# Orca0917/TransformerTTS

Measured on AMD Instinct MI355X. Metric: mel frames/sec teacher-forced step, LJSpeech-shape batch, 1/2/4/8 MI355X, higher is better.
Workload: dtype f32; 1 GPU; BASELINE configs[2] (batch 64, 1 GPU; per-GPU shard of configs[3]): training step (no-grad fwd + fwd + loss + bwd + clip + Adam), batch 64/GPU x 870 frames x 100 phonemes (dense), base config d_model 256, 3+3 layers, dropout on, fp32; global_batch=64, parallelism=dp1, batch_stream=one resident batch, accumulate=1, process_group=none, grad_allreduce=none (1 GPU), alignments_written=True, dma_gemms=True, layernorm_images=False, head_images=True, fused_cross_kv=True, wgrad_groups=True, twin_encoder=True, twin_postnet=True

## Files before the change

include/ttts_hip.h:

```cpp
#ifndef TTTS_HIP_H
#define TTTS_HIP_H

#include <stddef.h>
#include <stdint.h>

#ifdef __cplusplus
extern "C" {
#endif

#define TTTS_OK 0
#define TTTS_ERR_INVALID (-1)
#define TTTS_ERR_LAUNCH (-2)

#define TTTS_AMAX_SLOTS 1024

#define TTTS_ACT_NONE 0
#define TTTS_ACT_RELU 1
#define TTTS_ACT_TANH 2

typedef struct ttts_step_state {
    uint64_t seed;
    float lr;
    float p_tf;
    int64_t step;
// ... 46 lines not shown
int64_t ttts_weight_split_units(int64_t rows, int64_t cols, int mode, int channels_per_tap);
int ttts_weight_split_batched(const int64_t* descs, int n, int64_t total_blocks, void* stream);
int ttts_linear_fwd_x6(const float* x, const void* w_planes, const float* bias, const float* residual, float* y,
                       int64_t M, int N, int K, int act, float drop_p, uint64_t seed, const uint64_t* step_seed, int row_shift, int T,
                    void* stream);
int ttts_linear_fwd_h3(const float* x, const void* w_planes, const float* bias, const float* residual, float* y,
                       int64_t M, int N, int K, int act, float drop_p, uint64_t seed, const uint64_t* step_seed, int row_shift,
                       int T, const float* x_amax, float* y_amax_out, void* stream);
int ttts_conv1d_fwd_h3_bn_blocks(int B, int T, int cin, int cout, int taps);
int ttts_conv1d_fwd_h3_bn_chunk_rows(int B, int T, int cin, int cout, int taps);
int ttts_conv1d_fwd_h3(const float* x, const void* planes_fwd, const float* bias, float* y, int B, int T, int cin, int cout,
                       int taps, const float* x_amax, float* bn_partials, void* stream);
int ttts_amax_partials(const float* x, int64_t n, float* partials , void* stream);
int ttts_linear_bwd_data_h3(const float* dy, const void* wt_planes, const float* residual, float* dx, int64_t M, int N,
                            int K, const float* relu_out, float relu_scale, const float* dy_amax, float* dx_amax_out,
                            void* stream);
int ttts_act_image(const float* x, void* image, float* row_inv, int64_t M, int K, void* stream);
int ttts_linear_fwd_h3i(const void* x_image, const float* x_row_inv, const void* w_planes, const float* bias,
                        const float* residual, float* y, int64_t M, int N, int K, int act, float drop_p, uint64_t seed,
                        const uint64_t* step_seed, float* y_amax_out, void* stream);
int ttts_linear_bwd_data_h3i(const void* dy_image, const float* dy_row_inv, const void* wt_planes, const float* residual,
                             float* dx, int64_t M, int N, int K, const float* relu_out, float relu_scale,
                             float* dx_amax_out, void* stream);
int ttts_linear_fwd_h3d(const float* x, const void* w_planes, const float* bias, const float* residual, float* y,
                        int64_t M, int N, int K, int act, float drop_p, uint64_t seed, const uint64_t* step_seed,
                        const float* x_amax, float* y_amax_out, void* stream);
int ttts_linear_bwd_data_h3d(const float* dy, const void* wt_planes, const float* residual, float* dx, int64_t M, int N,
                             int K, const float* relu_out, float relu_scale, const float* dy_amax, float* dx_amax_out,
                             void* stream);
int ttts_linear_fwd_h3d_img(const float* x, const void* w_planes, const float* bias, void* y_image, float* y_row_inv,
                            int64_t M, int N, int K, const float* x_amax, float* y_amax_out, int amax_section_cols,
                            void* stream);
int ttts_head_image(const float* x, int64_t ld_x, void* image, int64_t ld_image, float* row_inv, int64_t M, int N, void* stream);
int ttts_conv1d_bwd_data_h3(const float* dy, const void* planes_bwd, float* dx, int B, int T, int cin, int cout, int taps,
                            const float* dy_amax, void* stream);
int ttts_linear_bwd_data_x6(const float* dy, const void* wt_planes, const float* residual, float* dx, int64_t M, int N,
                            int K, const float* relu_out, float relu_scale, void* stream);
int ttts_conv1d_fwd_x6(const float* x, const void* planes_fwd, const float* bias, float* y, int B, int T, int cin, int cout,
                       int taps, void* stream);
int ttts_conv1d_bwd_data_x6(const float* dy, const void* planes_bwd, float* dx, int B, int T, int cin, int cout, int taps,
                            void* stream);
int ttts_linear_bwd_weight_x6(const float* dy, const float* x, float* dw, float* dbias, float* ws, size_t ws_bytes,
                              int64_t M, int N, int K, int row_shift, int T, int accumulate, ttts_reduce_queue* queue,
                              void* stream);
int ttts_conv1d_bwd_weight_x6(const float* dy, const float* x, float* dw, float* dbias, float* ws, size_t ws_bytes, int B,
                              int T, int cin, int cout, int taps, int accumulate, ttts_reduce_queue* queue, void* stream);
int ttts_linear_bwd_weight_h3(const float* dy, const float* x, float* dw, float* dbias, float* ws, size_t ws_bytes,
                              int64_t M, int N, int K, int row_shift, int T, int accumulate, const float* dy_amax,
                              const float* x_amax, ttts_reduce_queue* queue, void* stream);
int ttts_conv1d_bwd_weight_h3(const float* dy, const float* x, float* dw, float* dbias, float* ws, size_t ws_bytes, int B,
                              int T, int cin, int cout, int taps, int accumulate, const float* dy_amax, const float* x_amax,
                              ttts_reduce_queue* queue, void* stream);
int ttts_wgrad_group_ok(int64_t M, int N, int K, int taps);
int ttts_wgrad_group(int n, const float* const* dy, const float* const* x, float* const* dw, float* const* dbias,
                     float* const* ws, const size_t* ws_bytes, const int64_t* M, const int* N, const int* K, const int* taps,
                     const int* T, const int* row_shift, int accumulate, const float* const* dy_amax, const float* const* x_amax,
                     ttts_reduce_queue* queue, void* stream);
int ttts_linear_bwd_weight_h3_parts(const float* dy, const float* x, float* const* dw_parts, float* const* dbias_parts, int nparts,
                                    float* ws, size_t ws_bytes, int64_t M, int N, int K, int accumulate, const float* dy_amax,
                                    const float* x_amax, ttts_reduce_queue* queue, void* stream);

size_t ttts_conv1d_pack_bytes(int cout, int cin, int taps);
int ttts_conv1d_pack_weight(const float* w, float* w_fwd, float* w_bwd, int cout, int cin, int taps, void* stream);
int ttts_conv1d_fwd(const float* x, const float* w_fwd, const float* bias, float* y, int B, int T, int cin, int cout,
                    int taps, void* stream);
int ttts_conv1d_bwd_data(const float* dy, const float* w_bwd, float* dx, int B, int T, int cin, int cout, int taps,
                         void* stream);
int ttts_conv1d_bwd_weight(const float* dy, const float* x, float* dw, float* dbias, float* ws, size_t ws_bytes, int B,
                           int T, int cin, int cout, int taps, int accumulate, ttts_reduce_queue* queue, void* stream);

size_t ttts_bn_workspace_bytes(int64_t M, int C);
int ttts_bn_train_stats(const float* x, float* mean, float* invstd, float* running_mean, float* running_var,
                        int64_t* num_batches_tracked, float* ws, size_t ws_bytes, int64_t M, int C, float momentum,
                        float eps, void* stream);
int ttts_bn_train_stats_from_partials(const float* partials, int nblk, float* mean, float* invstd, float* running_mean,
                                      float* running_var, int64_t* num_batches_tracked, int C, float momentum, float eps,
                                      void* stream);
int ttts_bn_train_stats_from_partials_rows(const float* partials, int nblk, const float* rows, int n_rows, float* mean,
                                           float* invstd, float* running_mean, float* running_var,
                                           int64_t* num_batches_tracked, int C, float momentum, float eps, void* stream);
int ttts_bn_train_stats_twin(const float* partials_a, int nblk_a, const float* rows_a, int n_rows_a, float* mean_a, float* invstd_a,
                             const float* partials_b, int nblk_b, const float* rows_b, int n_rows_b, float* mean_b, float* invstd_b,
                             float* running_mean, float* running_var, int64_t* num_batches_tracked, int C, float momentum,
                             float eps, void* stream);
int ttts_bn_eval_stats(const float* running_mean, const float* running_var, float* mean, float* invstd, int C, float eps,
                       void* stream);
int ttts_bn_apply_fwd(const float* x, const float* mean, const float* invstd, const float* gamma, const float* beta,
                      float* z, int64_t M, int C, int act, float drop_p, uint64_t seed, const uint64_t* step_seed,
                      float* z_amax_out, void* stream);
int ttts_bn_bwd(const float* dz, const float* x, const float* mean, const float* invstd, const float* gamma,
                const float* beta, float* dx, float* dgamma, float* dbeta, float* ws, size_t ws_bytes, int64_t M, int C,
                int act, float drop_p, uint64_t seed, const uint64_t* step_seed, int accumulate, float* dx_amax_out,
                int batch_stats, void* stream);

int ttts_layernorm_fwd(const float* x, const float* gamma, const float* beta, float* y, float* mean, float* rstd,
                       int64_t M, int d, float eps, float* y_amax_out ,
                       void* y_image_out, float* y_row_inv_out, void* stream);
size_t ttts_layernorm_bwd_workspace_bytes(int d);
int ttts_layernorm_bwd(const float* dy, const float* x, const float* mean, const float* rstd, const float* gamma,
                       float* dx, float* dgamma, float* dbeta, float* ws, size_t ws_bytes, int64_t M, int d,
                       int accumulate, void* dx_image_out ,
                       float* dx_row_inv_out, ttts_reduce_queue* queue, void* stream);
int ttts_layernorm_bwd_drop(const float* dy, const float* x, const float* mean, const float* rstd, const float* gamma,
                            float* dx, float* dgamma, float* dbeta, float* ws, size_t ws_bytes, int64_t M, int d,
                            int accumulate, float* dacc, float drop_p, uint64_t seed, const uint64_t* step_seed,
                            float* dacc_amax, void* dacc_image_out , float* dacc_row_inv_out,
// ... 268 lines not shown
```

transformertts_amd/_lib.py:

```python
from __future__ import annotations

import ctypes
import os
from ctypes import c_char_p, c_float, c_int, c_int64, c_size_t, c_uint64, c_void_p

import torch

_HERE = os.path.dirname(os.path.abspath(__file__))
LIB_PATH = os.environ.get("TTTS_LIB", os.path.join(_HERE, "libttts_hip.so"))

P, I, L, F, U, Z = c_void_p, c_int, c_int64, c_float, c_uint64, c_size_t

SIGNATURES = {
    "ttts_last_error": (c_char_p, []),
    "ttts_abi_version": (I, []),
    "ttts_linear_fwd": (I, [P, P, P, P, P, L, I, I, I, F, U, P, I, I, P]),
    "ttts_linear_bwd_data": (I, [P, P, P, P, L, I, I, P, F, P]),
    "ttts_wgrad_workspace_bytes": (Z, [L, I, I, I]),
    "ttts_linear_bwd_weight": (I, [P, P, P, P, P, Z, L, I, I, I, I, I, P, P]),
    "ttts_split_bytes": (Z, [L, L]),
    "ttts_split_image_bytes": (Z, [L, L, I, I, I]),
    "ttts_gemm_tile_choice": (I, [L, I, I, I]),
    "ttts_weight_split": (I, [P, P, I, I, I, I, I, P]),
    "ttts_weight_split_units": (L, [L, L, I, I]),
    "ttts_weight_split_batched": (I, [P, I, L, P]),
    "ttts_linear_fwd_x6": (I, [P, P, P, P, P, L, I, I, I, F, U, P, I, I, P]),
    "ttts_linear_fwd_h3": (I, [P, P, P, P, P, L, I, I, I, F, U, P, I, I, P, P, P]),
    "ttts_conv1d_fwd_h3": (I, [P, P, P, P, I, I, I, I, I, P, P, P]),
    "ttts_conv1d_fwd_h3_bn_blocks": (I, [I, I, I, I, I]),
    "ttts_conv1d_fwd_h3_bn_chunk_rows": (I, [I, I, I, I, I]),
    "ttts_bn_train_stats_from_partials": (I, [P, I, P, P, P, P, P, I, F, F, P]),
    "ttts_bn_train_stats_from_partials_rows": (I, [P, I, P, I, P, P, P, P, P, I, F, F, P]),
    "ttts_bn_train_stats_twin": (I, [P, I, P, I, P, P, P, I, P, I, P, P, P, P, P, I, F, F, P]),
    "ttts_amax_partials": (I, [P, L, P, P]),
    "ttts_linear_bwd_data_h3": (I, [P, P, P, P, L, I, I, P, F, P, P, P]),
    "ttts_act_image": (I, [P, P, P, L, I, P]),
    "ttts_linear_fwd_h3i": (I, [P, P, P, P, P, P, L, I, I, I, F, U, P, P, P]),
    "ttts_linear_bwd_data_h3i": (I, [P, P, P, P, P, L, I, I, P, F, P, P]),
    "ttts_linear_fwd_h3d": (I, [P, P, P, P, P, L, I, I, I, F, U, P, P, P, P]),
    "ttts_linear_bwd_data_h3d": (I, [P, P, P, P, L, I, I, P, F, P, P, P]),
    "ttts_linear_fwd_h3d_img": (I, [P, P, P, P, P, L, I, I, P, P, I, P]),
    "ttts_head_image": (I, [P, L, P, L, P, L, I, P]),
    "ttts_conv1d_bwd_data_h3": (I, [P, P, P, I, I, I, I, I, P, P]),
    "ttts_linear_bwd_data_x6": (I, [P, P, P, P, L, I, I, P, F, P]),
    "ttts_conv1d_fwd_x6": (I, [P, P, P, P, I, I, I, I, I, P]),
    "ttts_conv1d_bwd_data_x6": (I, [P, P, P, I, I, I, I, I, P]),
    "ttts_linear_bwd_weight_x6": (I, [P, P, P, P, P, Z, L, I, I, I, I, I, P, P]),
    "ttts_conv1d_bwd_weight_x6": (I, [P, P, P, P, P, Z, I, I, I, I, I, I, P, P]),
    "ttts_linear_bwd_weight_h3": (I, [P, P, P, P, P, Z, L, I, I, I, I, I, P, P, P, P]),
    "ttts_conv1d_bwd_weight_h3": (I, [P, P, P, P, P, Z, I, I, I, I, I, I, P, P, P, P]),
    "ttts_linear_bwd_weight_h3_parts": (I, [P, P, P, P, I, P, Z, L, I, I, I, P, P, P, P]),
    "ttts_wgrad_group_ok": (I, [L, I, I, I]),
    "ttts_wgrad_group": (I, [I, P, P, P, P, P, P, P, P, P, P, P, P, I, P, P, P, P]),
    "ttts_conv1d_pack_bytes": (Z, [I, I, I]),
    "ttts_conv1d_pack_weight": (I, [P, P, P, I, I, I, P]),
    "ttts_conv1d_fwd": (I, [P, P, P, P, I, I, I, I, I, P]),
    "ttts_conv1d_bwd_data": (I, [P, P, P, I, I, I, I, I, P]),
    "ttts_conv1d_bwd_weight": (I, [P, P, P, P, P, Z, I, I, I, I, I, I, P, P]),
    "ttts_bn_workspace_bytes": (Z, [L, I]),
    "ttts_bn_train_stats": (I, [P, P, P, P, P, P, P, Z, L, I, F, F, P]),
    "ttts_bn_eval_stats": (I, [P, P, P, P, I, F, P]),
    "ttts_bn_apply_fwd": (I, [P, P, P, P, P, P, L, I, I, F, U, P, P, P]),
    "ttts_bn_bwd": (I, [P, P, P, P, P, P, P, P, P, P, Z, L, I, I, F, U, P, I, P, I, P]),
    "ttts_layernorm_fwd": (I, [P, P, P, P, P, P, L, I, F, P, P, P, P]),
    "ttts_layernorm_bwd_workspace_bytes": (Z, [I]),
    "ttts_layernorm_bwd": (I, [P, P, P, P, P, P, P, P, P, Z, L, I, I, P, P, P, P]),
    "ttts_layernorm_bwd_drop": (I, [P, P, P, P, P, P, P, P, P, Z, L, I, I, P, F, U, P, P, P, P, P, P]),
    "ttts_attention_fwd": (I, [P, P, P, P, P, P, P, I, I, I, I, I, I, I, I, I, F, F, U, P, P]),
    "ttts_attention_fwd_x6": (I, [P, P, P, P, P, P, P, I, I, I, I, I, I, I, I, I, F, F, U, P, P]),
    "ttts_attention_fwd_h3": (I, [P, P, P, P, P, P, P, I, I, I, I, I, I, I, I, I, F, F, U, P, P, P, P, P, P, P]),
    "ttts_attention_bwd": (I, [P, P, P, P, P, P, P, P, P, P, P, I, I, I, I, I, I, I, I, I, I, I, I, F, F, U, P, P]),
    "ttts_attention_bwd_x6": (I, [P, P, P, P, P, P, P, P, P, P, P, I, I, I, I, I, I, I, I, I, I, I, I, F, F, U, P, P]),
    "ttts_attention_bwd_h3": (I, [P, P, P, P, P, P, P, P, P, P, P, I, I, I, I, I, I, I, I, I, I, I, I, F, F, U, P, P, P, P, P, P, P, P, P]),
    "ttts_attention_fwd_img": (I, [P, P, P, P, P, P, P, P, P, P, I, I, I, I, I, I, I, I, I, F, F, U, P, P, P, P, L, L, L, P]),
    "ttts_attention_bwd_img": (I, [P, P, P, P, P, P, P, P, P, P, P, P, P, P, I, I, I, I, I, I, I, I, I, I, I, I, F, F, U, P, P, P, P,
                                   P, I, L, L, L, P]),
    "ttts_attention_fwd_wide": (I, [P, P, P, P, P, P, P, I, I, I, I, I, I, I, I, I, F, F, U, P, P]),
    "ttts_attention_bwd_wide": (I, [P, P, P, P, P, P, P, P, P, P, P, I, I, I, I, I, I, I, I, I, I, I, I, F, F, U, P, P]),
    "ttts_attention_fwd_wide_masked": (I, [P, P, P, P, P, P, P, I, I, I, I, I, I, I, I, I, F, F, U, P, P, L, L, L, P, L, P]),
    "ttts_attention_bwd_wide_masked": (I, [P, P, P, P, P, P, P, P, P, P, P, I, I, I, I, I, I, I, I, I, I, I, I, F, F, U, P, P, L, L, L,
                                           P, L, P]),
    "ttts_attention_bwd_wide_dattn": (I, [P, P, P, P, P, P, P, P, P, P, P, I, I, I, I, I, I, I, I, I, I, I, I, F, F, U, P, P, L, L, L,
                                          P, L, P, P, L, L, L, P]),
    "ttts_guided_attention_fwd": (I, [P, P, P, U, F, I, I, I, I, P, I, I, I, P, P]),
    "ttts_guided_attention_bwd": (I, [P, P, P, U, F, I, I, I, I, I, I, P, P]),
    "ttts_alignment_rowstats": (I, [P, L, L, L, P, P, I, I, I, I, I, I, P, P, P, P]),
    "ttts_alignment_select": (I, [P, P, P, I, I, I, I, I, I, P, P, P]),
    "ttts_alignment_durations_argmax": (I, [P, P, P, P, I, I, I, I, I, P, P, P]),
    "ttts_alignment_mas_workspace_bytes": (Z, [I, I, I]),
    "ttts_alignment_mas": (I, [P, I, L, L, L, P, P, P, I, I, I, I, P, Z, P, P, P]),
    "ttts_dtw_workspace_bytes": (Z, [I, I, I]),
    "ttts_dtw": (I, [P, L, L, P, P, L, L, P, I, I, I, I, I, P, Z, P, P, P, P, P, P]),
    "ttts_audio_tables_bytes": (Z, [I, I, I]),
    "ttts_audio_tables_check": (I, [P, Z, I, I, I, I]),
    "ttts_logmel": (I, [P, L, P, I, I, I, I, I, I, P, F, P, P, P, I, P]),
    "ttts_logmel_stats": (I, [P, P, I, I, I, P, P]),
    "ttts_vocoder_pinv_check": (I, [P, Z, I, I]),
    "ttts_mel_to_magnitude": (I, [P, L, L, P, I, I, I, I, I, P, P, F, P, P, P]),
    "ttts_istft": (I, [P, P, I, I, I, I, P, P, P, P]),
    "ttts_stft_project": (I, [P, L, P, P, I, I, I, I, P, P, P, F, P, P, P]),
    "ttts_resample_table_bytes": (Z, [I, I]),
    "ttts_resample_table_check": (I, [P, Z, I, I, I]),
    "ttts_resample_tile": (I, []),
    "ttts_resample": (I, [P, L, P, I, I, I, I, I, P, P, L, P, P]),
    "ttts_pitch_lags": (I, []),
# ... 103 lines not shown
```

transformertts_amd/csrc/gemm.hip:

```cpp
#include <stdlib.h>

#include "gemm_common.h"

namespace ttts {

#ifndef TTTS_GEMM_BK
#define TTTS_GEMM_BK 16
#endif
#ifndef TTTS_X6_XCD
#define TTTS_X6_XCD 1
#endif
#ifndef TTTS_GEMM_MINWAVES
#define TTTS_GEMM_MINWAVES 3
#endif
constexpr int BK = TTTS_GEMM_BK;
constexpr int KC_LD = BK + 1;


template <int BM, int BN, int WM, int WN, bool A_KC, bool B_KC>
__global__ __launch_bounds__(256, TTTS_GEMM_MINWAVES) void gemm_f32_kernel(GemmArgs g) {
    const uint64_t seed_eff = site_seed(g.seed, g.step_seed);
    constexpr int WTM = BM / WM, WTN = BN / WN;
    constexpr int TM = WTM / 32, TN = WTN / 32;
    static_assert(WM * WN == 4, "4 waves per workgroup");
// ... 794 lines not shown
        for (int kt = kt_begin; kt < kt_end; ++kt) {
            const bool more = (kt + 1) < kt_end;
            if (more) load_tiles(kt + 1);
            compute(buf);
            if (more) store_tiles(buf ^ 1);
            __syncthreads();
            buf ^= 1;
        }
    }

    if (g.colsum != nullptr && blockIdx.x == 0 && ztap == 0) {
        float* fs = reinterpret_cast<float*>(lds);
        __syncthreads();
        if (a_slot) fs[a_rh * BM + a_col] = csum;
        __syncthreads();
        if (tid < BM && m0 + tid < g.M) g.colsum[(long)zsplit * g.M + m0 + tid] = fs[tid] + fs[BM + tid];
    }

    float* C = g.C + (long)z * g.c_zstride;
#pragma unroll
    for (int i = 0; i < TM; ++i)
#pragma unroll
        for (int j = 0; j < TN; ++j) {
            const int col = n0 + wn * WTN + j * 32 + l31;
            const int row0 = m0 + wm * WTM + i * 32;
#pragma unroll
            for (int r = 0; r < 16; ++r) {
                const int row = row0 + acc_row(r, half);
                if (row < g.M && col < g.N) C[(long)row * g.ldc + col] = acc[i][j][r];
            }
        }
}

template <int BM, int BN, int WM, int WN>
static int launch_wgrad_split(const GemmArgs& g, int zdim, hipStream_t stream) {
    dim3 grid(cdiv(g.N, BN), cdiv(g.M, BM), zdim);
    hipLaunchKernelGGL((wgrad_bf16x6_kernel<BM, BN, WM, WN>), grid, dim3(256), 0, stream, g);
    TTTS_LAUNCH_CHECK("wgrad_bf16x6_kernel");
    return TTTS_OK;
}

static int dispatch_wgrad_split(const GemmArgs& g, int zdim, int tile, hipStream_t stream) {
    switch (tile) {
        case TILE_64: return launch_wgrad_split<64, 64, 2, 2>(g, zdim, stream);
        case TILE_128x96: return launch_wgrad_split<128, 96, 4, 1>(g, zdim, stream);
        case TILE_96x128: return launch_wgrad_split<96, 128, 1, 4>(g, zdim, stream);
        default: return launch_wgrad_split<128, 128, 2, 2>(g, zdim, stream);
    }
}

enum WgradForm { WG_F32, WG_X6, WG_H3 };
struct WgradPlan { int tile; int nsplit; int kt_per_split; long tiles; };
struct WgradGroup { int cls; long tiles_total; long nkt_max; };

static long wgrad_target_single(WgradForm f, int tile, long tiles, long nkt) {
    if (f != WG_H3) return 768;
    if (tile == H3_TILE_256) return 256;
    return (tiles > 12 && nkt >= 800) ? 512 : 256;
}

constexpr long WG_GROUP_NKT512 = 200;
static long wgrad_group_many(int cls) { return (cls == 3 || cls == 4) ? 8 : 13; }
static long wgrad_target_group(const WgradGroup& grp) {
    if (grp.cls == 2) return 256;
    return (grp.tiles_total >= wgrad_group_many(grp.cls) && grp.nkt_max >= WG_GROUP_NKT512) ? 512 : 256;
}

static WgradPlan plan_wgrad(int64_t M, int N, int K, int taps, WgradForm f, const WgradGroup* grp = nullptr) {
    WgradPlan p; const long bk = f == WG_H3 ? HBK : BK, nkt = (M + bk - 1) / bk;
    p.tile = (K <= 96) ? TILE_128x96 : TILE_128;
    p.tiles = (long)cdiv(N, 128) * cdiv(K, 128) * taps;
    if (f != WG_F32) {
        if (N <= 64 && K <= 64) { p.tile = TILE_64; p.tiles = (long)cdiv(N, 64) * cdiv(K, 64) * taps; }
        else if (N <= 96 && K > 96) p.tile = TILE_96x128;
    } else if (p.tiles < 16) { p.tile = TILE_64; p.tiles = (long)cdiv(N, 64) * cdiv(K, 64) * taps; }
    if (f == WG_H3) {
        const long tiles256 = (long)cdiv(N, 256) * cdiv(K, 256) * taps;
        if (p.tile == TILE_128 && N >= 256 && K >= 256 && tiles256 >= 3 && nkt >= 800) { p.tile = H3_TILE_256; p.tiles = tiles256; }
    }
    long want = grp ? wgrad_target_group(*grp) / grp->tiles_total : wgrad_target_single(f, p.tile, p.tiles, nkt) / p.tiles;
    if (want < 1) want = 1;
    if (!grp && f != WG_F32 && want > 128) want = 128;
    if (want > nkt) want = nkt;
    long per = (nkt + want - 1) / want;
    if (per < 8 && nkt >= 8) per = 8;
    p.kt_per_split = (int)per;
    p.nsplit = (int)((nkt + per - 1) / per);
    return p;
}

static bool wgrad_use_x6(int N, int K) { return (N >= 128 || N == 80 || N == 96) && (K >= 128 || K == 80 || K == 96) && (N >= 128 || K >= 128); }

static int wgrad_class(int64_t M, int N, int K, int taps, long* tiles = nullptr) {
    if (!(M > 0 && N > 0 && K > 0 && taps >= 1 && taps <= 64 && N % 4 == 0 && K % 4 == 0 && wgrad_use_x6(N, K))) return 0;
    const WgradPlan p = plan_wgrad(M, N, K, taps, WG_H3);
    if (tiles) *tiles = p.tiles;
    if (p.tile == TILE_128) return 1;
    if (p.tile == H3_TILE_256 && N % 256 == 0 && K % 256 == 0) return 2;
    if (p.tile == TILE_128x96) return 3;
    if (p.tile == TILE_96x128) return 4;
    return 0;
}

struct WgradLayout { size_t colsum; size_t floats; };
static WgradLayout wgrad_layout(int nsplit, int N, int K, int taps) {
    const size_t prod = (size_t)nsplit * taps * N * K;
    return {prod, prod + (size_t)nsplit * N};
}

struct WgradProblem {
    const float *dy, *x; float* ws; size_t ws_bytes;
    int64_t M; int N, K, taps;
    int B, T, row_shift;
    const float *dy_amax, *x_amax;
    bool conv = false;
    bool bias = false;
};

static GemmArgs wgrad_args(const WgradProblem& pb, WgradForm f, const WgradPlan& p) {
    GemmArgs g = base_args();
    g.A = pb.dy; g.B = pb.x; g.C = pb.ws; g.M = pb.N; g.N = pb.K; g.K = (int)pb.M;
    g.lda = pb.N; g.ldb = pb.K; g.ldc = pb.K;
    g.a_bytes = (uint32_t)((uint64_t)pb.M * pb.N * 4); g.b_bytes = (uint32_t)((uint64_t)pb.M * pb.K * 4);
    g.T = (pb.conv || pb.row_shift != 0) ? pb.T : 0;
    g.shift0 = pb.conv ? -((pb.taps - 1) / 2) : pb.row_shift; g.shift_step = pb.conv ? 1 : 0;
    g.ztaps = pb.taps; g.kt_per_split = p.kt_per_split; g.c_zstride = (long)pb.N * pb.K;
    g.colsum = pb.bias ? pb.ws + wgrad_layout(p.nsplit, pb.N, pb.K, pb.taps).colsum : nullptr;
    if (f == WG_H3) {
        g.a_amax = pb.dy_amax; g.a_amax_n = H3_AMAX_PARTIALS;
        g.b_amax = pb.x_amax; g.b_amax_n = H3_AMAX_PARTIALS;
    }
    return g;
}

static int wgrad_reduce(const WgradProblem& pb, const WgradPlan& p, const float* colsum, float* const* dw, float* const* dbias, int nparts,
                        bool accumulate, hipStream_t stream, ttts_reduce_queue* queue) {
    if (pb.conv) {
        int rc = launch_conv_wgrad_reduce(pb.ws, dw[0], pb.N, pb.K, pb.taps, p.nsplit, accumulate, stream, queue);
        if (rc == TTTS_OK && colsum) rc = launch_reduce_rows(colsum, pb.N, p.nsplit, pb.N, dbias[0], pb.N, nullptr, accumulate, stream, queue);
        return rc;
    }
    const int Np = pb.N / nparts;
    const long nk = (long)pb.N * pb.K, np = (long)Np * pb.K;
    for (int i = 0; i < nparts; ++i) {
        int rc = launch_reduce_rows_pair(pb.ws + (size_t)i * np, nk, p.nsplit, np, dw[i], colsum ? colsum + (size_t)i * Np : nullptr, pb.N, Np,
                                         colsum ? dbias[i] : nullptr, accumulate, stream, queue);
        if (rc) return rc;
    }
    return TTTS_OK;
}

#define ENTRY_REQUIRE(cond, fmt, ...) TTTS_REQUIRE(cond, "%s: " fmt, name, ##__VA_ARGS__)
static int wgrad_check_operands(const char* name, const WgradProblem& pb) {
    ENTRY_REQUIRE(aligned16(pb.dy) && aligned16(pb.x) && aligned16(pb.ws), "pointers must be 16-byte aligned");
// ... 1 lines not shown
    return TTTS_OK;
}

enum WgradStage2 { WG_PAIR, WG_CONV, WG_PARTS };
static int wgrad_single(const char* name, WgradForm f, WgradStage2 stage, WgradProblem pb, float* const* dw, float* const* dbias,
                        int nparts, int accumulate, ttts_reduce_queue* queue, void* stream) {
    pb.conv = stage == WG_CONV;
    ENTRY_REQUIRE(pb.dy && pb.x && pb.ws && dw && (stage == WG_PARTS || dw[0]), "null pointer");
    ENTRY_REQUIRE(f != WG_H3 || (pb.dy_amax && pb.x_amax), "null pointer: dy_amax and x_amax (partial maxima of dy and x) are required");
    if (pb.conv) {
        ENTRY_REQUIRE(pb.B > 0 && pb.T > 0 && pb.K > 0 && pb.N > 0 && pb.taps > 0 && (pb.taps & 1), "bad dims B=%d T=%d cin=%d cout=%d taps=%d",
                      pb.B, pb.T, pb.K, pb.N, pb.taps);
        ENTRY_REQUIRE((long)pb.B * pb.T < (1L << 31), "B*T too large");
        pb.M = (int64_t)pb.B * pb.T;
    }
    ENTRY_REQUIRE(pb.M > 0 && pb.N > 0 && pb.K > 0 && pb.M < (1LL << 31), "bad dims M=%lld N=%d K=%d", (long long)pb.M, pb.N, pb.K);
    ENTRY_REQUIRE(pb.N % 4 == 0 && pb.K % 4 == 0, "%s=%d and %s=%d must be multiples of 4", pb.conv ? "cout" : "N", pb.N,
                  pb.conv ? "cin" : "K", pb.K);
    if (stage == WG_PARTS)
        ENTRY_REQUIRE(nparts > 0 && nparts <= 64 && pb.N % nparts == 0 && (pb.N / nparts) % 4 == 0,
                      "N=%d does not split in %d blocks of whole float4s", pb.N, nparts);
    if (int rc = wgrad_check_operands(name, pb)) return rc;
    ENTRY_REQUIRE(pb.ws_bytes >= ttts_wgrad_workspace_bytes(pb.M, pb.N, pb.K, pb.taps), "workspace too small");
    ENTRY_REQUIRE(pb.conv || pb.row_shift == 0 || (pb.T > 0 && pb.M % pb.T == 0), "row_shift needs T>0 and M %% T == 0");
    for (int i = 0; i < nparts; ++i) ENTRY_REQUIRE(dw[i] != nullptr, "null destination");
    if (!wgrad_use_x6(pb.N, pb.K)) f = WG_F32;
    pb.bias = dbias != nullptr && dbias[0] != nullptr;
    const WgradPlan p = plan_wgrad(pb.M, pb.N, pb.K, pb.taps, f);
    const GemmArgs g = wgrad_args(pb, f, p);
    const int zdim = p.nsplit * pb.taps;
    const int rc = f == WG_H3 ? dispatch_wgrad_h3(g, zdim, p.tile, (hipStream_t)stream)
           : f == WG_X6 ? dispatch_wgrad_split(g, zdim, p.tile, (hipStream_t)stream)
                        : dispatch_gemm<false, false>(g, zdim, p.tile, (hipStream_t)stream);
    return rc ? rc : wgrad_reduce(pb, p, g.colsum, dw, dbias, nparts, accumulate != 0, (hipStream_t)stream, queue);
}

}

using namespace ttts;

extern "C" {

size_t ttts_wgrad_workspace_bytes(int64_t M, int N, int K, int taps) {
    if (!(M > 0 && N > 0 && K > 0 && taps > 0)) return 0;
    int ns = 0;
    auto cover = [&](WgradForm f, const WgradGroup* grp) { const int n = plan_wgrad(M, N, K, taps, f, grp).nsplit; ns = n > ns ? n : ns; };
    cover(WG_F32, nullptr); cover(WG_X6, nullptr); cover(WG_H3, nullptr);
    long tiles = 0;
    if (const int cls = wgrad_class(M, N, K, taps, &tiles)) {
        const long many = wgrad_group_many(cls);
        const WgradGroup alone = {cls, tiles, (long)((M + HBK - 1) / HBK)}, full = {cls, tiles < many ? many : tiles, WG_GROUP_NKT512};
        cover(WG_H3, &alone); cover(WG_H3, &full);
    }
    return wgrad_layout(ns, N, K, taps).floats * sizeof(float);
}

int ttts_linear_bwd_weight(const float* dy, const float* x, float* dw, float* dbias, float* ws, size_t ws_bytes,
                           int64_t M, int N, int K, int row_shift, int T, int accumulate, ttts_reduce_queue* queue, void* stream) {
    return wgrad_single("linear_bwd_weight", WG_F32, WG_PAIR, {dy, x, ws, ws_bytes, M, N, K, 1, 0, T, row_shift, nullptr, nullptr}, &dw, &dbias, 1,
                        accumulate, queue, stream);
}
int ttts_linear_bwd_weight_x6(const float* dy, const float* x, float* dw, float* dbias, float* ws, size_t ws_bytes,
                              int64_t M, int N, int K, int row_shift, int T, int accumulate, ttts_reduce_queue* queue, void* stream) {
    return wgrad_single("linear_bwd_weight_x6", WG_X6, WG_PAIR, {dy, x, ws, ws_bytes, M, N, K, 1, 0, T, row_shift, nullptr, nullptr}, &dw, &dbias, 1,
                        accumulate, queue, stream);
}
int ttts_linear_bwd_weight_h3(const float* dy, const float* x, float* dw, float* dbias, float* ws, size_t ws_bytes,
                              int64_t M, int N, int K, int row_shift, int T, int accumulate, const float* dy_amax,
                              const float* x_amax, ttts_reduce_queue* queue, void* stream) {
    return wgrad_single("linear_bwd_weight_h3", WG_H3, WG_PAIR, {dy, x, ws, ws_bytes, M, N, K, 1, 0, T, row_shift, dy_amax, x_amax}, &dw, &dbias, 1,
                        accumulate, queue, stream);
}

int ttts_linear_bwd_weight_h3_parts(const float* dy, const float* x, float* const* dw_parts, float* const* dbias_parts, int nparts,
                                    float* ws, size_t ws_bytes, int64_t M, int N, int K, int accumulate, const float* dy_amax,
                                    const float* x_amax, ttts_reduce_queue* queue, void* stream) {
    return wgrad_single("linear_bwd_weight_h3_parts", WG_H3, WG_PARTS, {dy, x, ws, ws_bytes, M, N, K, 1, 0, 0, 0, dy_amax, x_amax}, dw_parts,
                        dbias_parts, nparts, accumulate, queue, stream);
}

int ttts_conv1d_bwd_weight(const float* dy, const float* x, float* dw, float* dbias, float* ws, size_t ws_bytes, int B,
                           int T, int cin, int cout, int taps, int accumulate, ttts_reduce_queue* queue, void* stream) {
    return wgrad_single("conv1d_bwd_weight", WG_F32, WG_CONV, {dy, x, ws, ws_bytes, 0, cout, cin, taps, B, T, 0, nullptr, nullptr}, &dw, &dbias, 1,
                        accumulate, queue, stream);
}
int ttts_conv1d_bwd_weight_x6(const float* dy, const float* x, float* dw, float* dbias, float* ws, size_t ws_bytes, int B,
                              int T, int cin, int cout, int taps, int accumulate, ttts_reduce_queue* queue, void* stream) {
    return wgrad_single("conv1d_bwd_weight_x6", WG_X6, WG_CONV, {dy, x, ws, ws_bytes, 0, cout, cin, taps, B, T, 0, nullptr, nullptr}, &dw, &dbias, 1,
                        accumulate, queue, stream);
}
int ttts_conv1d_bwd_weight_h3(const float* dy, const float* x, float* dw, float* dbias, float* ws, size_t ws_bytes, int B,
                              int T, int cin, int cout, int taps, int accumulate, const float* dy_amax, const float* x_amax,
                              ttts_reduce_queue* queue, void* stream) {
    return wgrad_single("conv1d_bwd_weight_h3", WG_H3, WG_CONV, {dy, x, ws, ws_bytes, 0, cout, cin, taps, B, T, 0, dy_amax, x_amax}, &dw, &dbias, 1,
                        accumulate, queue, stream);
}

int ttts_wgrad_group_ok(int64_t M, int N, int K, int taps) { return wgrad_class(M, N, K, taps); }

int ttts_wgrad_group(int n, const float* const* dy, const float* const* x, float* const* dw, float* const* dbias,
                     float* const* ws, const size_t* ws_bytes, const int64_t* M, const int* N, const int* K, const int* taps,
                     const int* T, const int* row_shift, int accumulate, const float* const* dy_amax, const float* const* x_amax,
                     ttts_reduce_queue* queue, void* stream_) {
    const char* name = "wgrad_group";
    hipStream_t stream = (hipStream_t)stream_;
    ENTRY_REQUIRE(n >= 1 && n <= WG_GROUP_MAX && dy && x && dw && ws && ws_bytes && M && N && K && taps && T && row_shift && dy_amax && x_amax,
                  "bad arguments");
    WgradProblem pb[WG_GROUP_MAX]; WgradPlan plan[WG_GROUP_MAX]; GemmArgs gs[WG_GROUP_MAX]; int zd[WG_GROUP_MAX];
    WgradGroup grp = {wgrad_class(M[0], N[0], K[0], taps[0]), 0, 0};
    for (int i = 0; i < n; ++i) {
        pb[i] = {dy[i], x[i], ws[i], ws_bytes[i], M[i], N[i], K[i], taps[i], 0, T[i], row_shift[i], dy_amax[i], x_amax[i], taps[i] > 1,
                 dbias != nullptr && dbias[i] != nullptr};
        ENTRY_REQUIRE(dy[i] && x[i] && dw[i] && ws[i] && dy_amax[i] && x_amax[i], "null pointer (member %d)", i);
        ENTRY_REQUIRE(taps[i] <= 1 || (taps[i] & 1), "member %d: bad dims M=%lld N=%d K=%d taps=%d (a convolution's tap count must be odd)", i,
                      (long long)M[i], N[i], K[i], taps[i]);
        long tiles = 0;
        ENTRY_REQUIRE(grp.cls != 0 && wgrad_class(M[i], N[i], K[i], taps[i], &tiles) == grp.cls && M[i] < (1LL << 31),
                      "member %d (M=%lld N=%d K=%d taps=%d) is not of the group's class %d", i, (long long)M[i], N[i], K[i], taps[i], grp.cls);
        if (int rc = wgrad_check_operands(name, pb[i])) return rc;
        grp.tiles_total += tiles;
        if ((M[i] + HBK - 1) / HBK > grp.nkt_max) grp.nkt_max = (M[i] + HBK - 1) / HBK;
    }
    for (int i = 0; i < n; ++i) {
        plan[i] = plan_wgrad(M[i], N[i], K[i], taps[i], WG_H3, &grp);
        ENTRY_REQUIRE(ws_bytes[i] >= wgrad_layout(plan[i].nsplit, N[i], K[i], taps[i]).floats * sizeof(float), "workspace %d too small", i);
        ENTRY_REQUIRE((taps[i] == 1 && row_shift[i] == 0) || (T[i] > 0 && M[i] % T[i] == 0 && (grp.cls != 2 || T[i] >= 16)),
                      "member %d: a convolution / a shifted linear needs its utterance length", i);
        ENTRY_REQUIRE(taps[i] == 1 || row_shift[i] == 0, "member %d: a convolution takes no row shift of its own", i);
        gs[i] = wgrad_args(pb[i], WG_H3, plan[i]);
        zd[i] = plan[i].nsplit * taps[i];
    }
    int rc = grp.cls == 2 ? launch_wgrad_dma_group(gs, zd, n, stream) : launch_wgrad_h3_group(gs, zd, n, plan[0].tile, stream);
    for (int i = 0; i < n && rc == TTTS_OK; ++i)
        rc = wgrad_reduce(pb[i], plan[i], gs[i].colsum, dw + i, dbias ? dbias + i : nullptr, 1, accumulate != 0, stream, queue);
    return rc;
}
#undef ENTRY_REQUIRE

size_t ttts_conv1d_pack_bytes(int cout, int cin, int taps) { return (size_t)cout * cin * taps * sizeof(float); }

int ttts_conv1d_pack_weight(const float* w, float* w_fwd, float* w_bwd, int cout, int cin, int taps, void* stream) {
    TTTS_REQUIRE(w && (w_fwd || w_bwd), "conv1d_pack_weight: null pointer");
    long n = (long)cout * cin * taps;
    hipLaunchKernelGGL(conv_pack_weight_kernel, dim3(cdiv(n, 256)), dim3(256), 0, (hipStream_t)stream, w, w_fwd, w_bwd,
                       cout, cin, taps);
    TTTS_LAUNCH_CHECK("conv_pack_weight_kernel");
    return TTTS_OK;
}

int ttts_gemm_tile_choice(int64_t M, int N, int K, int x6) {
    if (x6 == 2) return h3_tile_choice(M, N, K);
    if (N <= 96 && (long)cdiv(M, 128) >= 384) return TILE_128x96;
    return choose_tile(M, N, 1, x6 != 0);
}

size_t ttts_split_bytes(int64_t rows, int64_t cols) { return (size_t)3 * (size_t)rows * (size_t)cols * 2; }

size_t ttts_split_image_bytes(int64_t rows, int64_t cols, int mode, int channels_per_tap, int taps) {
    if (mode < 4) return ttts_split_bytes(rows, cols);
    const bool conv = h3_mode_base(mode) >= 2;
    return h3_plane_bytes(rows, h3_image_cols(cols, conv ? channels_per_tap : 0, conv ? taps : 0)) + 16;
}

int ttts_weight_split(const float* w, void* planes, int rows, int cols, int mode, int channels_per_tap, int taps,
                      void* stream) {
    TTTS_REQUIRE(w && planes && rows > 0 && cols > 0, "weight_split: bad arguments");
    TTTS_REQUIRE(mode >= 0 && mode <= 11, "weight_split: mode must be 0..11");
    TTTS_REQUIRE(cols % (mode >= 4 ? 4 : BK) == 0, "weight_split: cols=%d must be a multiple of %d", cols, mode >= 4 ? 4 : BK);
    TTTS_REQUIRE((mode < 4 ? mode : h3_mode_base(mode)) < 2 || (channels_per_tap > 0 && taps > 0 && cols == channels_per_tap * taps),
                 "weight_split: conv modes need cols == channels_per_tap * taps");
// ... 232 lines not shown
```

transformertts_amd/csrc/gemm_common.h:

```cpp
#pragma once
#include "ttts_common.h"

namespace ttts {

struct GemmArgs {
    const float* A;
    const float* B;
    float* C;
    int M, N, K;
    long lda, ldb, ldc;
    int T;
    int cin;
    int shift0, shift_step;
    int ztaps;
    int kt_per_split;
    long c_zstride;
    const float* bias;
    int act;
    float drop_scale;
    uint32_t drop_thr;
    uint64_t seed;
    const uint64_t* step_seed;
    const float* residual;
    long ldr;
// ... 191 lines not shown
            for (int idx = tid; idx < 32 * run; idx += 256) {
                const int rr = idx / run, j = idx - rr * run, cc = j / tcn, tt = j - cc * tcn;
                t[tt][rr][cc] = (rr < nr && cc < nc) ? w[((long)(r0 + rr) * c2 + ch0 + cc) * taps + tc0 + tt] : 0.f;
            }
        } else {
            for (int idx = tid; idx < 32 * run; idx += 256) {
                const int cc = idx / run, j = idx - cc * run, rr = j / tcn, tt = j - rr * tcn;
                t[tt][rr][cc] = (rr < nr && cc < nc) ? w[((long)(ch0 + cc) * R + r0 + rr) * taps + tc0 + tt] : 0.f;
            }
        }
        __syncthreads();
        const int rr = tid >> 3, q = (tid & 7) * 4;
        if (rr < nr) {
            for (int tt = 0; tt < tcn; ++tt) {
                const int cp = c_off + (mode >= 2 ? (tc0 + tt) * padc : 0) + ch0 + q;
                unsigned short h[4], l[4];
#pragma unroll
                for (int e = 0; e < 4; ++e) {
                    const float v = t[tt][rr][q + e] * w_scale;
                    const _Float16 hh = (_Float16)v;
                    const _Float16 ll = (_Float16)(v - (float)hh);
                    h[e] = __builtin_bit_cast(unsigned short, hh);
                    l[e] = __builtin_bit_cast(unsigned short, ll);
                }
                const long o = k16 ? ((long)(cp >> 4) * Rimg + r_off + r0 + rr) * 32 + (cp & 15)
                                   : ((long)(cp >> 5) * 2 * Rimg + r_off + r0 + rr) * 32 + (cp & 31);
                *reinterpret_cast<uint2*>(planes + o) = make_uint2(h[0] | ((uint32_t)h[1] << 16), h[2] | ((uint32_t)h[3] << 16));
                *reinterpret_cast<uint2*>(planes + o + (k16 ? 16L : (long)Rimg * 32)) =
                    make_uint2(l[0] | ((uint32_t)l[1] << 16), l[2] | ((uint32_t)l[3] << 16));
            }
        }
        __syncthreads();
    }
    }
}

enum { TILE_AUTO = 0, TILE_64 = 1, TILE_128 = 2, TILE_64x128 = 3, TILE_128x96 = 4, TILE_96x128 = 5,
       H3_TILE_256 = 6, H3_TILE_256x128 = 7,
       H3_TILE_256x128_PAIR = 8 };

bool h3_supports(const GemmArgs& g);
int h3_tile_choice(long M, long N, long K);
void launch_weight_split_h3(const float* w, void* planes, int rows, int cols, int mode, int c2, int taps, hipStream_t stream,
                            bool k16 = false);
int dispatch_h3(const GemmArgs& g, hipStream_t stream);
int h3_bn_blocks(long M, long N, long K);
int h3_bn_chunk_rows(long M, long N, long K);
int dispatch_wgrad_h3(const GemmArgs& g, int zdim, int tile, hipStream_t stream);
__device__ __forceinline__ int xcd_renumber(int bid, int total) {
    const int per = total >> 3, rem = total & 7;
    const int xcd = bid & 7, slot = bid >> 3;
    return xcd * per + min(xcd, rem) + slot;
}
constexpr int WG_GROUP_MAX = 4;
struct WgradGroupArgs {
    GemmArgs g[WG_GROUP_MAX];
    int first[WG_GROUP_MAX + 1];
    int n;
};
int launch_wgrad_h3_group(const GemmArgs* gs, const int* zdims, int n, int tile, hipStream_t stream);
bool wgrad_dma_supports(const GemmArgs& g, int tile);
int launch_wgrad_dma(const GemmArgs& g, int zdim, hipStream_t stream);
int launch_wgrad_dma_group(const GemmArgs* gs, const int* zdims, int n, hipStream_t stream);
bool h3i_supports(const GemmArgs& g);
int dispatch_h3i(const GemmArgs& g, hipStream_t stream);

}
```

transformertts_amd/ops.py:

```python
from __future__ import annotations

import os
import weakref
from ctypes import c_void_p
from typing import NamedTuple, Optional

import torch

from . import _lib

ACT_NONE, ACT_RELU, ACT_TANH = 0, 1, 2
AMAX_SLOTS = 1024


def _p(t: Optional[torch.Tensor]):
    return None if t is None else c_void_p(t.data_ptr())


_raw_stream = getattr(torch._C, "_cuda_getCurrentRawStream", None)


def _stream():
    if _raw_stream is not None:
        return c_void_p(_raw_stream(torch.cuda.current_device()))
# ... 214 lines not shown
    def take(self, n: int = 1):
        if not self.clean or self.next + n > self.SLICES:
            return None
        self.next += n
        return self.buf[self.next - 1] if n == 1 else self.buf[self.next - n:self.next]


_amax_arenas = {}


_pass_id = [0]


def amax_arena_reset(device) -> None:
    _pass_id[0] += 1
    arena = _amax_arenas.get(device)
    if arena is None:
        arena = _amax_arenas[device] = _AmaxArena(device)
    arena.reset()


def amax_arena_release(device) -> None:
    arena = _amax_arenas.get(device)
    if arena is not None:
        arena.clean = False


def _amax_slots(device, zero: bool) -> torch.Tensor:
    if zero:
        arena = _amax_arenas.get(device)
        got = arena.take() if arena is not None else None
        if got is not None:
            return got
    a = _guarded(1, AMAX_SLOTS, device, "amax slots")[0] if GUARD else torch.empty(AMAX_SLOTS, dtype=torch.float32, device=device)
    if zero:
        _lib.check(_lib.load().ttts_zero(_p(a), AMAX_SLOTS * 4, _stream()), "ttts_zero")
    return a


def _amax_slots_n(device, n: int) -> torch.Tensor:
    arena = _amax_arenas.get(device)
    got = arena.take(n) if arena is not None else None
    if got is not None:
        return got.view(n, AMAX_SLOTS)
    a = _guarded(n, AMAX_SLOTS, device, "section maxima") if GUARD else torch.empty(n, AMAX_SLOTS, dtype=torch.float32, device=device)
    _lib.check(_lib.load().ttts_zero(_p(a), a.numel() * 4, _stream()), "ttts_zero")
    return a


DEFER_REDUCE = True


WGRAD_GROUPS = True
WGRAD_GROUP_MAX = 4
WGRAD_GROUP_SIZE = {1: 4, 2: 3, 3: 2, 4: 2}
WGRAD_SIDE_STREAM = False
WGRAD_SIDE_MAX_ROWS = 0


class WgradMember(NamedTuple):
    dy: torch.Tensor
    dy_amax: torch.Tensor
    x: torch.Tensor
    x_amax: torch.Tensor
    dw: torch.Tensor
    db: Optional[torch.Tensor]
    M: int
    N: int
    K: int
    ws: torch.Tensor
    taps: int
    T: int
    row_shift: int


class ReduceQueue:

    def __init__(self):
        self._lib = _lib.load()
        self.handle = c_void_p(self._lib.ttts_reduce_queue_create())
        if not self.handle:
            raise MemoryError("ttts_reduce_queue_create failed")
        self.keep: list = []
        self.wg = {1: [], 2: [], 3: [], 4: []}
        self._armed = False
        self._side = None
        self._side_busy = False

    def _arm(self) -> None:
        if not self._armed:
            torch.autograd.Variable._execution_engine.queue_callback(self._final)
            self._armed = True

    def arg(self, ws: torch.Tensor):
        self._arm()
        self.keep.append(ws)
        return self.handle

    def defer_wgrad(self, cls: int, dy, dy_am, x, x_am, dw, db, M: int, N: int, K: int, taps: int = 1, T: int = 0,
                    row_shift: int = 0) -> None:
        if taps > 1 and taps % 2 == 0:
            raise ValueError(f"defer_wgrad: a convolution's tap count must be odd (taps={taps})")
        self._arm()
        pend = self.wg[cls]
        if pend and (pend[0].M != M or pend[0].dy.device != dy.device):
            self.launch_wgrads(cls)
            pend = self.wg[cls]
        ws = _ws(self._lib.ttts_wgrad_workspace_bytes(M, N, K, taps), x.device)
        pend.append(WgradMember(dy, dy_am, x, x_am, dw, db, M, N, K, ws, taps, T, row_shift))
        if len(pend) >= WGRAD_GROUP_SIZE[cls]:
            self.launch_wgrads(cls)

    def launch_wgrads(self, cls: int = 0) -> None:
        if cls == 0:
            for c in (1, 2, 3, 4):
                self.launch_wgrads(c)
            return
        if not self.wg[cls]:
            return
        import ctypes
        wg, self.wg[cls] = self.wg[cls], []
        n = len(wg)
        PA, ZA, LA, IA = ctypes.c_void_p * n, ctypes.c_size_t * n, ctypes.c_int64 * n, ctypes.c_int * n
        ptr = lambda ts: PA(*[(t.data_ptr() if t is not None else None) for t in ts])
        dy, dy_amax, x, x_amax, dw, db, M, N, K, ws, taps, T, row_shift = zip(*wg)

        def go(stream):
            _lib.check(self._lib.ttts_wgrad_group(
                n, ptr(dy), ptr(x), ptr(dw), ptr(db), ptr(ws), ZA(*[w.numel() * 4 for w in ws]), LA(*M), IA(*N), IA(*K), IA(*taps),
                IA(*T), IA(*row_shift), 1, ptr(dy_amax), ptr(x_amax), self.handle if DEFER_REDUCE else None, stream), "ttts_wgrad_group")
        if WGRAD_SIDE_STREAM and DEFER_REDUCE and (WGRAD_SIDE_MAX_ROWS <= 0 or M[0] <= WGRAD_SIDE_MAX_ROWS):
            dev = dy[0].device
            if self._side is None or self._side.device != dev:
                self._side = torch.cuda.Stream(device=dev)
            cur = torch.cuda.current_stream(dev)
            self._side.wait_stream(cur)
            with torch.cuda.stream(self._side):
                go(c_void_p(self._side.cuda_stream))
            self._side_busy = True
            self.keep.extend(t for m in wg for t in (m.dy, m.dy_amax, m.x, m.x_amax))
        else:
            go(_stream())
        self.keep.extend(ws)

    def join_side(self) -> None:
        if self._side_busy:
            torch.cuda.current_stream(self._side.device).wait_stream(self._side)
            self._side_busy = False

    def _final(self) -> None:
        self._armed = False
        self.flush()

    def pending(self) -> int:
        return int(self._lib.ttts_reduce_queue_pending(self.handle))

    def flush(self) -> None:
        self.launch_wgrads()
        self.join_side()
        if self.keep or self.pending():
            _lib.check(self._lib.ttts_reduce_queue_flush(self.handle, _stream()), "ttts_reduce_queue_flush")
            self.keep.clear()

    def clear(self) -> None:
        _lib.check(self._lib.ttts_reduce_queue_clear(self.handle), "ttts_reduce_queue_clear")
        self.join_side()
        self.keep.clear()
        self.wg = {1: [], 2: [], 3: [], 4: []}
        self._armed = False

    def __del__(self):
        try:
            if self.handle:
                self._lib.ttts_reduce_queue_destroy(self.handle)
                self.handle = None
        except Exception:
            pass

# ... 1858 lines not shown
```

Measured before the change: 4.051 million mel frames/s.

## Let eligible class-1 weight-gradient GEMMs join pending class-2 groups as guests

Weight-gradient GEMMs of class 1 with large row counts and 256-divisible dims can now be added as guests to a pending class-2 group, so they run in the same grouped launch with 256 tiles. Group capacity grows to 8 members, and workspace sizing covers the hosted plan. The aim is fewer launches and better CU fill from merging small groups. The cost is a larger kernel argument struct and possible load imbalance or changed tile choice for the guests.

```diff
diff --git a/include/ttts_hip.h b/include/ttts_hip.h
--- a/include/ttts_hip.h
+++ b/include/ttts_hip.h
@@ -122,6 +122,7 @@
                               int T, int cin, int cout, int taps, int accumulate, const float* dy_amax, const float* x_amax,
                               ttts_reduce_queue* queue, void* stream);
 int ttts_wgrad_group_ok(int64_t M, int N, int K, int taps);
+int ttts_wgrad_group_guest_ok(int64_t M, int N, int K, int taps);
 int ttts_wgrad_group(int n, const float* const* dy, const float* const* x, float* const* dw, float* const* dbias,
                      float* const* ws, const size_t* ws_bytes, const int64_t* M, const int* N, const int* K, const int* taps,
                      const int* T, const int* row_shift, int accumulate, const float* const* dy_amax, const float* const* x_amax,
diff --git a/transformertts_amd/_lib.py b/transformertts_amd/_lib.py
--- a/transformertts_amd/_lib.py
+++ b/transformertts_amd/_lib.py
@@ -51,6 +51,7 @@
     "ttts_conv1d_bwd_weight_h3": (I, [P, P, P, P, P, Z, I, I, I, I, I, I, P, P, P, P]),
     "ttts_linear_bwd_weight_h3_parts": (I, [P, P, P, P, I, P, Z, L, I, I, I, P, P, P, P]),
     "ttts_wgrad_group_ok": (I, [L, I, I, I]),
+    "ttts_wgrad_group_guest_ok": (I, [L, I, I, I]),
     "ttts_wgrad_group": (I, [I, P, P, P, P, P, P, P, P, P, P, P, P, I, P, P, P, P]),
     "ttts_conv1d_pack_bytes": (Z, [I, I, I]),
     "ttts_conv1d_pack_weight": (I, [P, P, P, I, I, I, P]),
diff --git a/transformertts_amd/csrc/gemm.hip b/transformertts_amd/csrc/gemm.hip
--- a/transformertts_amd/csrc/gemm.hip
+++ b/transformertts_amd/csrc/gemm.hip
@@ -870,6 +870,7 @@
 enum WgradForm { WG_F32, WG_X6, WG_H3 };
 struct WgradPlan { int tile; int nsplit; int kt_per_split; long tiles; };
 struct WgradGroup { int cls; long tiles_total; long nkt_max; };
+constexpr long WG_TILE256_NKT = 800;
 
 static long wgrad_target_single(WgradForm f, int tile, long tiles, long nkt) {
     if (f != WG_H3) return 768;
@@ -894,7 +895,8 @@
     } else if (p.tiles < 16) { p.tile = TILE_64; p.tiles = (long)cdiv(N, 64) * cdiv(K, 64) * taps; }
     if (f == WG_H3) {
         const long tiles256 = (long)cdiv(N, 256) * cdiv(K, 256) * taps;
-        if (p.tile == TILE_128 && N >= 256 && K >= 256 && tiles256 >= 3 && nkt >= 800) { p.tile = H3_TILE_256; p.tiles = tiles256; }
+        if (p.tile == TILE_128 && N >= 256 && K >= 256 && tiles256 >= 3 && nkt >= WG_TILE256_NKT) { p.tile = H3_TILE_256; p.tiles = tiles256; }
+        if (grp && grp->cls == 2 && p.tile == TILE_128 && N % 256 == 0 && K % 256 == 0) { p.tile = H3_TILE_256; p.tiles = tiles256; }
     }
     long want = grp ? wgrad_target_group(*grp) / grp->tiles_total : wgrad_target_single(f, p.tile, p.tiles, nkt) / p.tiles;
     if (want < 1) want = 1;
@@ -918,6 +920,10 @@
     if (p.tile == TILE_128x96) return 3;
     if (p.tile == TILE_96x128) return 4;
     return 0;
+}
+
+static bool wgrad_guest_ok(int64_t M, int N, int K, int taps) {
+    return taps == 1 && N % 256 == 0 && K % 256 == 0 && wgrad_class(M, N, K, taps) == 1 && (M + HBK - 1) / HBK >= WG_TILE256_NKT;
 }
 
 struct WgradLayout { size_t colsum; size_t floats; };
@@ -1025,6 +1031,10 @@
         const WgradGroup alone = {cls, tiles, (long)((M + HBK - 1) / HBK)}, full = {cls, tiles < many ? many : tiles, WG_GROUP_NKT512};
         cover(WG_H3, &alone); cover(WG_H3, &full);
     }
+    if (wgrad_guest_ok(M, N, K, taps)) {
+        const WgradGroup hosted = {2, 3 + (long)(N / 256) * (K / 256), (long)((M + HBK - 1) / HBK)};
+        cover(WG_H3, &hosted);
+    }
     return wgrad_layout(ns, N, K, taps).floats * sizeof(float);
 }
 
@@ -1070,6 +1080,7 @@
 }
 
 int ttts_wgrad_group_ok(int64_t M, int N, int K, int taps) { return wgrad_class(M, N, K, taps); }
+int ttts_wgrad_group_guest_ok(int64_t M, int N, int K, int taps) { return wgrad_guest_ok(M, N, K, taps) ? 1 : 0; }
 
 int ttts_wgrad_group(int n, const float* const* dy, const float* const* x, float* const* dw, float* const* dbias,
                      float* const* ws, const size_t* ws_bytes, const int64_t* M, const int* N, const int* K, const int* taps,
@@ -1080,7 +1091,12 @@
     ENTRY_REQUIRE(n >= 1 && n <= WG_GROUP_MAX && dy && x && dw && ws && ws_bytes && M && N && K && taps && T && row_shift && dy_amax && x_amax,
                   "bad arguments");
     WgradProblem pb[WG_GROUP_MAX]; WgradPlan plan[WG_GROUP_MAX]; GemmArgs gs[WG_GROUP_MAX]; int zd[WG_GROUP_MAX];
+    ENTRY_REQUIRE(n <= WG_GROUP_MAX_128 || wgrad_class(M[0], N[0], K[0], taps[0]) == 2 || wgrad_guest_ok(M[0], N[0], K[0], taps[0]),
+                  "bad arguments: %d members (more than %d: class 2 and its guests only)", n, WG_GROUP_MAX_128);
     WgradGroup grp = {wgrad_class(M[0], N[0], K[0], taps[0]), 0, 0};
+    for (int i = 1; i < n && grp.cls != 2; ++i)
+        if (wgrad_class(M[i], N[i], K[i], taps[i]) == 2) grp.cls = 2;
+    ENTRY_REQUIRE(n <= WG_GROUP_MAX_128 || grp.cls == 2, "bad arguments: %d members and none of class 2 (guests need a host)", n);
     for (int i = 0; i < n; ++i) {
         pb[i] = {dy[i], x[i], ws[i], ws_bytes[i], M[i], N[i], K[i], taps[i], 0, T[i], row_shift[i], dy_amax[i], x_amax[i], taps[i] > 1,
                  dbias != nullptr && dbias[i] != nullptr};
@@ -1088,7 +1104,10 @@
         ENTRY_REQUIRE(taps[i] <= 1 || (taps[i] & 1), "member %d: bad dims M=%lld N=%d K=%d taps=%d (a convolution's tap count must be odd)", i,
                       (long long)M[i], N[i], K[i], taps[i]);
         long tiles = 0;
-        ENTRY_REQUIRE(grp.cls != 0 && wgrad_class(M[i], N[i], K[i], taps[i], &tiles) == grp.cls && M[i] < (1LL << 31),
+        const int own = wgrad_class(M[i], N[i], K[i], taps[i], &tiles);
+        const bool guest = grp.cls == 2 && own == 1 && wgrad_guest_ok(M[i], N[i], K[i], taps[i]);
+        if (guest) tiles = (long)(N[i] / 256) * (K[i] / 256);
+        ENTRY_REQUIRE(grp.cls != 0 && (own == grp.cls || guest) && M[i] < (1LL << 31),
                       "member %d (M=%lld N=%d K=%d taps=%d) is not of the group's class %d", i, (long long)M[i], N[i], K[i], taps[i], grp.cls);
         if (int rc = wgrad_check_operands(name, pb[i])) return rc;
         grp.tiles_total += tiles;
diff --git a/transformertts_amd/csrc/gemm_common.h b/transformertts_amd/csrc/gemm_common.h
--- a/transformertts_amd/csrc/gemm_common.h
+++ b/transformertts_amd/csrc/gemm_common.h
@@ -267,12 +267,14 @@
     const int xcd = bid & 7, slot = bid >> 3;
     return xcd * per + min(xcd, rem) + slot;
 }
-constexpr int WG_GROUP_MAX = 4;
+constexpr int WG_GROUP_MAX = 8;
+constexpr int WG_GROUP_MAX_128 = 4;
 struct WgradGroupArgs {
     GemmArgs g[WG_GROUP_MAX];
     int first[WG_GROUP_MAX + 1];
     int n;
 };
+static_assert(sizeof(WgradGroupArgs) <= 4096, "WgradGroupArgs outgrew the kernel-argument limit");
 int launch_wgrad_h3_group(const GemmArgs* gs, const int* zdims, int n, int tile, hipStream_t stream);
 bool wgrad_dma_supports(const GemmArgs& g, int tile);
 int launch_wgrad_dma(const GemmArgs& g, int zdim, hipStream_t stream);
diff --git a/transformertts_amd/ops.py b/transformertts_amd/ops.py
--- a/transformertts_amd/ops.py
+++ b/transformertts_amd/ops.py
@@ -290,8 +290,10 @@
 
 
 WGRAD_GROUPS = True
-WGRAD_GROUP_MAX = 4
+WGRAD_GROUP_MAX = 8
 WGRAD_GROUP_SIZE = {1: 4, 2: 3, 3: 2, 4: 2}
+WGRAD_GUESTS = True
+WGRAD_GUEST_MIN_ROWS = 55680
 WGRAD_SIDE_STREAM = False
 WGRAD_SIDE_MAX_ROWS = 0
 
@@ -310,6 +312,7 @@
     taps: int
     T: int
     row_shift: int
+    guest: bool = False
 
 
 class ReduceQueue:
@@ -340,13 +343,18 @@
         if taps > 1 and taps % 2 == 0:
             raise ValueError(f"defer_wgrad: a convolution's tap count must be odd (taps={taps})")
         self._arm()
+        host = self.wg[2]
+        guest = bool(cls == 1 and WGRAD_GUESTS and host and M >= WGRAD_GUEST_MIN_ROWS and row_shift == 0 and host[0].M == M and
+                     host[0].dy.device == dy.device and self._lib.ttts_wgrad_group_guest_ok(M, N, K, taps))
+        if guest:
+            cls = 2
         pend = self.wg[cls]
         if pend and (pend[0].M != M or pend[0].dy.device != dy.device):
             self.launch_wgrads(cls)
             pend = self.wg[cls]
         ws = _ws(self._lib.ttts_wgrad_workspace_bytes(M, N, K, taps), x.device)
-        pend.append(WgradMember(dy, dy_am, x, x_am, dw, db, M, N, K, ws, taps, T, row_shift))
-        if len(pend) >= WGRAD_GROUP_SIZE[cls]:
+        pend.append(WgradMember(dy, dy_am, x, x_am, dw, db, M, N, K, ws, taps, T, row_shift, guest))
+        if sum(not m.guest for m in pend) >= WGRAD_GROUP_SIZE[cls] or len(pend) >= WGRAD_GROUP_MAX:
             self.launch_wgrads(cls)
 
     def launch_wgrads(self, cls: int = 0) -> None:
@@ -356,12 +364,19 @@
             return
         if not self.wg[cls]:
             return
+        wg, self.wg[cls] = self.wg[cls], []
+        if all(m.guest for m in wg):
+            for i in range(0, len(wg), WGRAD_GROUP_SIZE[1]):
+                self._launch_group(wg[i:i + WGRAD_GROUP_SIZE[1]])
+            return
+        self._launch_group(wg)
+
+    def _launch_group(self, wg) -> None:
         import ctypes
-        wg, self.wg[cls] = self.wg[cls], []
         n = len(wg)
         PA, ZA, LA, IA = ctypes.c_void_p * n, ctypes.c_size_t * n, ctypes.c_int64 * n, ctypes.c_int * n
         ptr = lambda ts: PA(*[(t.data_ptr() if t is not None else None) for t in ts])
-        dy, dy_amax, x, x_amax, dw, db, M, N, K, ws, taps, T, row_shift = zip(*wg)
+        dy, dy_amax, x, x_amax, dw, db, M, N, K, ws, taps, T, row_shift, _ = zip(*wg)
 
         def go(stream):
             _lib.check(self._lib.ttts_wgrad_group(
```

After: 4.081 million mel frames/s, median of 6. Within noise of the previous version (+0.7%).
